# Kamino666/video_features

Hardware: NVIDIA H100
Metric: frames/sec CLIP-ViT-B/32 @224px (higher is better)
Workload: dtype f16

## Files before the change

### video_features_b200/csrc/common.cuh

```cuda
#pragma once
#include <cuda.h>
#include <cuda_runtime.h>
#include <cuda_fp16.h>
#include <stdint.h>

namespace vf {

__device__ __forceinline__ uint32_t smem_u32(const void* p) {
    return static_cast<uint32_t>(__cvta_generic_to_shared(p));
}

__device__ __forceinline__ void mbar_init(uint64_t* bar, uint32_t count) {
    asm volatile("mbarrier.init.shared::cta.b64 [%0], %1;" ::"r"(smem_u32(bar)), "r"(count));
}
__device__ __forceinline__ void fence_mbar_init() {
    asm volatile("fence.mbarrier_init.release.cluster;" ::: "memory");
}
__device__ __forceinline__ void mbar_expect_tx(uint64_t* bar, uint32_t bytes) {
    asm volatile("mbarrier.arrive.expect_tx.shared::cta.b64 _, [%0], %1;" ::"r"(smem_u32(bar)), "r"(bytes)
                 : "memory");
}
__device__ __forceinline__ void mbar_arrive(uint64_t* bar) {
    asm volatile("mbarrier.arrive.shared::cta.b64 _, [%0];" ::"r"(smem_u32(bar)) : "memory");
}
__device__ __forceinline__ void mbar_wait(uint64_t* bar, uint32_t parity) {
    asm volatile(
        "{\n"
        ".reg .pred P1;\n"
        "LAB_WAIT:\n"
        "mbarrier.try_wait.parity.shared::cta.b64 P1, [%0], %1;\n"
        "@P1 bra DONE;\n"
        "bra LAB_WAIT;\n"
        "DONE:\n"
        "}" ::"r"(smem_u32(bar)),
        "r"(parity)
        : "memory");
}

__device__ __forceinline__ void tma_prefetch_desc(const CUtensorMap* tm) {
    asm volatile("prefetch.tensormap [%0];" ::"l"(reinterpret_cast<uint64_t>(tm)) : "memory");
}
__device__ __forceinline__ void tma_load_2d(void* smem_dst, const CUtensorMap* tm, uint64_t* bar, int c0, int c1) {
    asm volatile(
        "cp.async.bulk.tensor.2d.shared::cluster.global.mbarrier::complete_tx::bytes [%0], [%1, {%3, %4}], [%2];" ::"r"(
            smem_u32(smem_dst)),
        "l"(reinterpret_cast<uint64_t>(tm)), "r"(smem_u32(bar)), "r"(c0), "r"(c1)
        : "memory");
}
__device__ __forceinline__ void tma_load_4d(void* smem_dst, const CUtensorMap* tm, uint64_t* bar, int c0, int c1,
                                            int c2, int c3) {
    asm volatile(
        "cp.async.bulk.tensor.4d.shared::cluster.global.mbarrier::complete_tx::bytes [%0], [%1, {%3, %4, %5, %6}], "
        "[%2];" ::"r"(smem_u32(smem_dst)),
        "l"(reinterpret_cast<uint64_t>(tm)), "r"(smem_u32(bar)), "r"(c0), "r"(c1), "r"(c2), "r"(c3)
        : "memory");
}
__device__ __forceinline__ void tma_load_5d(void* smem_dst, const CUtensorMap* tm, uint64_t* bar, int c0, int c1,
                                            int c2, int c3, int c4) {
    asm volatile(
        "cp.async.bulk.tensor.5d.shared::cluster.global.mbarrier::complete_tx::bytes [%0], [%1, {%3, %4, %5, %6, "
        "%7}], [%2];" ::"r"(smem_u32(smem_dst)),
        "l"(reinterpret_cast<uint64_t>(tm)), "r"(smem_u32(bar)), "r"(c0), "r"(c1), "r"(c2), "r"(c3), "r"(c4)
        : "memory");
}

__device__ __forceinline__ void tma_store_2d(const CUtensorMap* tm, const void* smem_src, int c0, int c1) {
    asm volatile("cp.async.bulk.tensor.2d.global.shared::cta.bulk_group [%0, {%2, %3}], [%1];" ::"l"(
                     reinterpret_cast<uint64_t>(tm)),
                 "r"(smem_u32(smem_src)), "r"(c0), "r"(c1)
                 : "memory");
}
__device__ __forceinline__ void tma_reduce_add_2d(const CUtensorMap* tm, const void* smem_src, int c0, int c1) {
    asm volatile("cp.reduce.async.bulk.tensor.2d.global.shared::cta.add.tile.bulk_group [%0, {%2, %3}], [%1];" ::"l"(
                     reinterpret_cast<uint64_t>(tm)),
                 "r"(smem_u32(smem_src)), "r"(c0), "r"(c1)
                 : "memory");
}
__device__ __forceinline__ void red_add_f32x4(float* gptr, float4 v) {
    asm volatile("red.global.add.v4.f32 [%0], {%1, %2, %3, %4};" ::"l"(gptr), "f"(v.x), "f"(v.y), "f"(v.z), "f"(v.w) : "memory");
}
__device__ __forceinline__ void bulk_commit() { asm volatile("cp.async.bulk.commit_group;" ::: "memory"); }
template <int N>
__device__ __forceinline__ void bulk_wait_read() {
    asm volatile("cp.async.bulk.wait_group.read %0;" ::"n"(N) : "memory");
}
template <int N>
__device__ __forceinline__ void bulk_wait() {
    asm volatile("cp.async.bulk.wait_group %0;" ::"n"(N) : "memory");
}
__device__ __forceinline__ void st_shared_b32(uint32_t addr, uint32_t v) {
    asm volatile("st.shared.b32 [%0], %1;" ::"r"(addr), "r"(v) : "memory");
}
__device__ __forceinline__ void st_shared_v2_f32(uint32_t addr, float x, float y) {
    asm volatile("st.shared.v2.f32 [%0], {%1, %2};" ::"r"(addr), "f"(x), "f"(y) : "memory");
}
__device__ __forceinline__ void fence_proxy_async() { asm volatile("fence.proxy.async.shared::cta;" ::: "memory"); }
__device__ __forceinline__ void named_bar_sync(uint32_t id, uint32_t nthreads) {
    asm volatile("bar.sync %0, %1;" ::"r"(id), "r"(nthreads) : "memory");
}
__device__ __forceinline__ void named_bar_arrive(uint32_t id, uint32_t nthreads) {
    asm volatile("bar.arrive %0, %1;" ::"r"(id), "r"(nthreads) : "memory");
}
template <uint32_t N>
__device__ __forceinline__ void setmaxnreg_dec() {
    asm volatile("setmaxnreg.dec.sync.aligned.u32 %0;" ::"n"(N));
}
template <uint32_t N>
__device__ __forceinline__ void setmaxnreg_inc() {
    asm volatile("setmaxnreg.inc.sync.aligned.u32 %0;" ::"n"(N));
}

__device__ __forceinline__ uint64_t wgmma_desc_sw128(const void* smem_tile) {
    uint64_t d = 0;
    d |= static_cast<uint64_t>((smem_u32(smem_tile) & 0x3FFFF) >> 4);
    d |= static_cast<uint64_t>(1) << 16;
    d |= static_cast<uint64_t>(1024 >> 4) << 32;
    d |= static_cast<uint64_t>(1) << 62;
    return d;
}
__device__ __forceinline__ void wgmma_fence() { asm volatile("wgmma.fence.sync.aligned;" ::: "memory"); }
__device__ __forceinline__ void wgmma_commit() { asm volatile("wgmma.commit_group.sync.aligned;" ::: "memory"); }
template <int N>
__device__ __forceinline__ void wgmma_wait() {
    asm volatile("wgmma.wait_group.sync.aligned %0;" ::"n"(N) : "memory");
}
template <int R>
__device__ __forceinline__ void wgmma_fence_regs(float* d) {
#pragma unroll
    for (int i = 0; i < R; ++i) asm volatile("" : "+f"(d[i])::"memory");
}

__device__ __forceinline__ float warp_sum(float v) {
#pragma unroll
    for (int o = 16; o > 0; o >>= 1) v += __shfl_xor_sync(0xffffffffu, v, o);
    return v;
}
__device__ __forceinline__ float warp_max(float v) {
#pragma unroll
    for (int o = 16; o > 0; o >>= 1) v = fmaxf(v, __shfl_xor_sync(0xffffffffu, v, o));
    return v;
}
__device__ __forceinline__ uint32_t pack_half2(float a, float b) {
    __half2 h = __floats2half2_rn(a, b);
    return *reinterpret_cast<uint32_t*>(&h);
}

}
```

### video_features_b200/csrc/gemm.cu

```cuda
#include "gemm_kernel.cuh"

namespace vf {

extern template int launch_bn<1, false, true>(GEMM_LAUNCH_ARGS);
extern template int launch_bn<1, true, true>(GEMM_LAUNCH_ARGS);
extern template int launch_bn<1, false, false>(GEMM_LAUNCH_ARGS);
extern template int launch_bn<1, true, false>(GEMM_LAUNCH_ARGS);
extern template int launch_bn<2, false, false>(GEMM_LAUNCH_ARGS);
extern template int launch_bn<2, true, false>(GEMM_LAUNCH_ARGS);

namespace {

typedef CUresult (*EncodeTiledFn)(CUtensorMap*, CUtensorMapDataType, cuuint32_t, void*, const cuuint64_t*,
                                  const cuuint64_t*, const cuuint32_t*, const cuuint32_t*, CUtensorMapInterleave,
                                  CUtensorMapSwizzle, CUtensorMapL2promotion, CUtensorMapFloatOOBfill);

EncodeTiledFn get_encode_tiled() {
    static EncodeTiledFn fn = nullptr;
    if (fn) return fn;
    void* p = nullptr;
    cudaDriverEntryPointQueryResult q;
    if (cudaGetDriverEntryPoint("cuTensorMapEncodeTiled", &p, cudaEnableDefault, &q) != cudaSuccess ||
        q != cudaDriverEntryPointSuccess)
        return nullptr;
    fn = reinterpret_cast<EncodeTiledFn>(p);
    return fn;
}

}

int device_sm_count() {
    static std::atomic<int> sms[64];
    int dev = 0;
    if (cudaGetDevice(&dev) != cudaSuccess || dev < 0 || dev >= 64) return 132;
    int v = sms[dev].load(std::memory_order_relaxed);
    if (v == 0) {
        if (cudaDeviceGetAttribute(&v, cudaDevAttrMultiProcessorCount, dev) != cudaSuccess || v <= 0) v = 132;
        sms[dev].store(v, std::memory_order_relaxed);
    }
    return v;
}

int make_tmap_2d(CUtensorMap* out, const void* base, int elem_bytes, uint64_t rows, uint64_t cols,
                 uint64_t row_pitch_bytes, uint32_t box_rows, uint32_t box_cols) {
    EncodeTiledFn enc = get_encode_tiled();
    if (!enc) return fail(VF_ERR_CUDA, "cuTensorMapEncodeTiled entry point unavailable (no CUDA driver?)");
    if ((reinterpret_cast<uintptr_t>(base) & 15) || (row_pitch_bytes & 15))
        return fail(VF_ERR_INVALID, "TMA operand must be 16-byte aligned with a 16-byte multiple row pitch");
    if (box_cols * uint32_t(elem_bytes) != 128) return fail(VF_ERR_INVALID, "TMA box rows must be 128 bytes");
    const CUtensorMapDataType dt = elem_bytes == 2 ? CU_TENSOR_MAP_DATA_TYPE_FLOAT16 : CU_TENSOR_MAP_DATA_TYPE_FLOAT32;
    cuuint64_t dims[2] = {cols, rows};
    cuuint64_t strides[1] = {row_pitch_bytes};
    cuuint32_t box[2] = {box_cols, box_rows};
    cuuint32_t estr[2] = {1, 1};
    CUresult r = enc(out, dt, 2, const_cast<void*>(base), dims, strides, box, estr, CU_TENSOR_MAP_INTERLEAVE_NONE,
                     CU_TENSOR_MAP_SWIZZLE_128B, CU_TENSOR_MAP_L2_PROMOTION_L2_256B, CU_TENSOR_MAP_FLOAT_OOB_FILL_NONE);
    if (r != CUDA_SUCCESS) return fail(VF_ERR_CUDA, "cuTensorMapEncodeTiled failed with CUresult %d", int(r));
    return VF_OK;
}

struct GemmProf {
    bool on = false;
    std::vector<cudaEvent_t> ev;
    size_t used = 0;
    double flops = 0.0;
};
static thread_local GemmProf g_prof;

template <bool PP>
static int run_gemm_launch(const CUtensorMap& tmA, const CUtensorMap& tmB, const CUtensorMap& tmD,
                           const CUtensorMap& tmD2, int bn, const GemmEpi& ep, int M, int N, const ConvGeom& cg,
                           cudaStream_t stream) {
    const bool split = ep.split_off > 0 && !ep.out_f32;
    if constexpr (!PP) {
        if (cg.nsplit == 2)
            return split ? launch_bn<2, true, PP>(tmA, tmB, tmD, tmD2, bn, ep, M, N, cg, stream)
                         : launch_bn<2, false, PP>(tmA, tmB, tmD, tmD2, bn, ep, M, N, cg, stream);
    }
    return split ? launch_bn<1, true, PP>(tmA, tmB, tmD, tmD2, bn, ep, M, N, cg, stream)
                 : launch_bn<1, false, PP>(tmA, tmB, tmD, tmD2, bn, ep, M, N, cg, stream);
}

static int run_gemm(const CUtensorMap& tmA, bool pp, const __half* B, int ldb, int64_t Ktot, int M, int N,
                    const ConvGeom& cg, const GemmEpi& ep, cudaStream_t stream) {
    if (!ep.out) return fail(VF_ERR_INVALID, "gemm: null output");
    if (reinterpret_cast<uintptr_t>(ep.out) & 15) return fail(VF_ERR_INVALID, "gemm: output must be 16-byte aligned");
    if (ep.accumulate && !ep.out_f32) return fail(VF_ERR_INVALID, "gemm: accumulate needs fp32 output");
    if (N % 8) return fail(VF_ERR_INVALID, "gemm: N=%d must be a multiple of 8", N);
    if (ep.act < VF_ACT_NONE || ep.act > VF_ACT_GELU) return fail(VF_ERR_INVALID, "gemm: unknown activation %d", ep.act);
    if (ep.out_f32 ? (ep.ldo % 4) : (ep.ldo % 8)) return fail(VF_ERR_INVALID, "gemm: ldo breaks 16-byte rows");
    if (ep.split_off && (ep.out_f32 || ep.split_off < N || ep.split_off % 8))
        return fail(VF_ERR_INVALID, "gemm: split output needs fp16 out and split_off >= N, multiple of 8");
    const int bm = tile_rows(pp);
    const int64_t num_m = (M + bm - 1) / bm, sms = device_sm_count();
    int bn = 256;
    int64_t best = INT64_MAX;
    for (int cand : {256, 192, 128, 64}) {
        const int64_t cost = (num_m * ((N + cand - 1) / cand) + sms - 1) / sms * cand;
        if (cost < best) { best = cost; bn = cand; }
    }
    CUtensorMap tmB, tmD, tmD2;
    VF_TRY(make_tmap_2d(&tmB, B, 2, uint64_t(N), uint64_t(Ktot), uint64_t(ldb) * 2, uint32_t(bn), BK));
    const int eb = ep.out_f32 ? 4 : 2;
    VF_TRY(make_tmap_2d(&tmD, ep.out, eb, uint64_t(M), uint64_t(N), uint64_t(ep.ldo) * eb, EPI_ROWS, 128 / eb));
    if (ep.split_off)
        VF_TRY(make_tmap_2d(&tmD2, static_cast<__half*>(ep.out) + ep.split_off, eb, uint64_t(M), uint64_t(N),
                            uint64_t(ep.ldo) * eb, EPI_ROWS, 128 / eb));
    else
        tmD2 = tmD;
    auto launch = [&] {
        return pp ? run_gemm_launch<true>(tmA, tmB, tmD, tmD2, bn, ep, M, N, cg, stream)
                  : run_gemm_launch<false>(tmA, tmB, tmD, tmD2, bn, ep, M, N, cg, stream);
    };
    if (!g_prof.on) return launch();
    if (g_prof.used + 2 > g_prof.ev.size())
        for (int i = 0; i < 2; ++i) {
            cudaEvent_t e;
            VF_CUDA(cudaEventCreate(&e));
            g_prof.ev.push_back(e);
        }
    VF_CUDA(cudaEventRecord(g_prof.ev[g_prof.used], stream));
    const int st = launch();
    VF_CUDA(cudaEventRecord(g_prof.ev[g_prof.used + 1], stream));
    g_prof.used += 2;
    double kexec = double(Ktot);
    if (cg.nsplit == 2 && cg.lo_mask) {
        const int kpt = (cg.k_per_tap + BK - 1) / BK;
        int skipped = 0;
        for (int kk = 0; kk < kpt && kk < 64; ++kk) skipped += int((cg.lo_mask >> kk) & 1ull);
        kexec -= double(cg.ntaps) * skipped * BK;
    }
    g_prof.flops += 2.0 * double(M) * double(N) * kexec;
    return st;
}

bool gemm_profile_on() { return g_prof.on; }
int gemm_profile(int enable) {
    g_prof.on = enable != 0;
    return VF_OK;
}
int gemm_profile_read(double* ms, int64_t* launches, double* flops) {
    VF_CUDA(cudaDeviceSynchronize());
    double t = 0.0;
    for (size_t i = 0; i + 1 < g_prof.used; i += 2) {
        float x = 0.f;
        VF_CUDA(cudaEventElapsedTime(&x, g_prof.ev[i], g_prof.ev[i + 1]));
        t += x;
    }
    if (ms) *ms = t;
    if (launches) *launches = int64_t(g_prof.used / 2);
    if (flops) *flops = g_prof.flops;
    g_prof.used = 0;
    g_prof.flops = 0.0;
    return VF_OK;
}

int gemm_f16(const __half* A, int lda, const __half* B, int ldb, int M, int N, int K, const GemmEpi& ep,
             cudaStream_t stream) {
    if (M <= 0 || N <= 0 || K <= 0) return fail(VF_ERR_INVALID, "gemm: empty problem %dx%dx%d", M, N, K);
    if (K % 8 || lda % 8 || ldb % 8) return fail(VF_ERR_INVALID, "gemm: K/lda/ldb must be multiples of 8");
    ConvGeom cg;
    memset(&cg, 0, sizeof(cg));
    cg.ntaps = 1;
    cg.k_per_tap = K;
    cg.nsplit = 1;
    CUtensorMap tmA;
    VF_TRY(make_tmap_2d(&tmA, A, 2, uint64_t(M), uint64_t(K), uint64_t(lda) * 2, tile_rows(true), BK));
    return run_gemm(tmA, true, B, ldb, K, M, N, cg, ep, stream);
}

int conv_gemm_f16(const __half* X, int C, int64_t P, const __half* Wt, int N, const ConvGeom& g, const GemmEpi& ep,
                  cudaStream_t stream) {
    if (P <= 0 || P > 0x7fffffff || N <= 0 || C <= 0) return fail(VF_ERR_INVALID, "conv_gemm: bad size");
    if (C % 8) return fail(VF_ERR_INVALID, "conv_gemm: C=%d must be a multiple of 8", C);
    if (g.ntaps < 1 || g.ntaps > 64 || g.k_per_tap < 8 || g.k_per_tap % 8)
        return fail(VF_ERR_INVALID, "conv_gemm: bad tap geometry (%d taps x %d)", g.ntaps, g.k_per_tap);
    if (g.nsplit != 1 && g.nsplit != 2) return fail(VF_ERR_INVALID, "conv_gemm: nsplit must be 1 or 2");
    const int kpt = (g.k_per_tap + BK - 1) / BK;
    if (g.lo_mask && (kpt > 64 || (kpt < 64 && (g.lo_mask >> kpt) != 0)))
        return fail(VF_ERR_INVALID, "conv_gemm: lo_mask 0x%llx names K blocks beyond the %d of a tap", g.lo_mask, kpt);
    if (g.mask && (g.Tp < 1 || g.Hp < 1 || g.Wp < 1 || g.row0 < 0))
        return fail(VF_ERR_INVALID, "conv_gemm: bad mask volume %dx%dx%d, row0 %d", g.Tp, g.Hp, g.Wp, g.row0);
    CUtensorMap tmA;
    VF_TRY(make_tmap_2d(&tmA, X, 2, uint64_t(P), uint64_t(g.k_per_tap), uint64_t(C) * 2, tile_rows(false), BK));
    const int64_t Ktot = int64_t(g.ntaps) * g.k_per_tap * g.nsplit;
    if (Ktot % 8) return fail(VF_ERR_INVALID, "conv_gemm: K must be a multiple of 8");
    return run_gemm(tmA, false, Wt, int(Ktot), Ktot, int(P), N, g, ep, stream);
}

}
```

### video_features_b200/csrc/gemm_inst_pp.cu

```cuda
#include "gemm_kernel.cuh"

namespace vf {
template int launch_bn<1, false, true>(GEMM_LAUNCH_ARGS);
template int launch_bn<1, true, true>(GEMM_LAUNCH_ARGS);
}
```

### video_features_b200/csrc/gemm_kernel.cuh

```cuda
#pragma once
#include <stdarg.h>
#include <stdlib.h>
#include <string.h>

#include <atomic>
#include <vector>

#include "common.cuh"
#include "internal.h"
#include "wgmma.cuh"

namespace vf {

namespace {

constexpr int BK = 64;
constexpr int THREADS = 384;
constexpr uint32_t PRODUCER_REGS = 40, CONSUMER_REGS = 232;
constexpr int EPI_ROWS = 64;
constexpr uint32_t STG_BYTES = EPI_ROWS * 128;
constexpr uint32_t STAGING_BYTES = 2 * 2 * STG_BYTES;
constexpr uint32_t SMEM_LIMIT = 227 * 1024;
constexpr uint32_t MAX_STAGES = 8;
constexpr uint32_t RING_BUDGET = SMEM_LIMIT - STAGING_BYTES - 2 * MAX_STAGES * 8 - 1024;

template <int BN, int NSPLIT, bool PP>
struct GemmCfg {
    static constexpr int BM = PP ? 64 : 128;
    static constexpr uint32_t A_BYTES = BM * BK * 2;
    static constexpr uint32_t B_TILE = BN * BK * 2;
    static constexpr uint32_t B_BYTES = NSPLIT * B_TILE;
    static constexpr uint32_t STAGE_BYTES = A_BYTES + B_BYTES;
    static constexpr int STAGES = RING_BUDGET / STAGE_BYTES > MAX_STAGES ? MAX_STAGES : int(RING_BUDGET / STAGE_BYTES);
    static constexpr uint32_t BAR_BYTES = 2 * STAGES * 8;
    static constexpr uint32_t SMEM_BYTES = STAGES * STAGE_BYTES + STAGING_BYTES + BAR_BYTES + 1024;
    static_assert(STAGES >= 2, "at least two pipeline stages");
    static_assert(SMEM_BYTES <= SMEM_LIMIT, "shared memory budget");
    static_assert(A_BYTES % 1024 == 0 && B_TILE % 1024 == 0, "swizzle-128B tiles must stay 1024-byte aligned");
};

constexpr int tile_rows(bool pp) { return pp ? GemmCfg<64, 1, true>::BM : GemmCfg<64, 1, false>::BM; }

template <int ACT>
__device__ __forceinline__ float apply_act(float v) {
    if (ACT == VF_ACT_QUICKGELU) {
        return __fdividef(v, 1.0f + __expf(-1.702f * v));
    } else if (ACT == VF_ACT_RELU) {
        return fmaxf(v, 0.0f);
    } else if (ACT == VF_ACT_SIGMOID) {
        return __fdividef(1.0f, 1.0f + __expf(-v));
    } else if (ACT == VF_ACT_TANH) {
        return 1.0f - __fdividef(2.0f, 1.0f + __expf(2.0f * v));
    } else if (ACT == VF_ACT_LEAKY) {
        return v > 0.0f ? v : __fmul_rn(v, 0.1f);
    } else if (ACT == VF_ACT_GELU) {
        return 0.5f * v * (1.0f + erff(v * 0.70710678118654752f));
    }
    return v;
}

template <int BN, int NSPLIT, bool SPLIT, bool PP, int ACT>
__global__ void __launch_bounds__(THREADS, 1)
gemm_f16_kernel(const __grid_constant__ CUtensorMap tmA, const __grid_constant__ CUtensorMap tmB,
                const __grid_constant__ CUtensorMap tmD, const __grid_constant__ CUtensorMap tmD2, const GemmEpi ep,
                const int M, const int N, const __grid_constant__ ConvGeom cg) {
    using Cfg = GemmCfg<BN, NSPLIT, PP>;
    static_assert(PP ? NSPLIT == 1 : true, "split weights run in the conv mode only");
    constexpr int STAGES = Cfg::STAGES;
    constexpr int BM = Cfg::BM;
    extern __shared__ uint8_t smem_raw[];
    uint8_t* smem = reinterpret_cast<uint8_t*>((reinterpret_cast<uintptr_t>(smem_raw) + 1023) & ~uintptr_t(1023));
    uint8_t* sA = smem;
    uint8_t* sB = smem + STAGES * Cfg::A_BYTES;
    uint8_t* sD = smem + STAGES * Cfg::STAGE_BYTES;
    uint64_t* full = reinterpret_cast<uint64_t*>(sD + STAGING_BYTES);
    uint64_t* empty = full + STAGES;

    const int warp = threadIdx.x >> 5;
    const int lane = threadIdx.x & 31;
    const int num_m = (M + BM - 1) / BM;
    const int num_n = (N + BN - 1) / BN;
    const int num_tiles = num_m * num_n;
    auto tile_m0 = [&](int tile) { return (PP ? tile / num_n : tile % num_m) * BM; };
    auto tile_n0 = [&](int tile) { return (PP ? tile % num_n : tile / num_m) * BN; };
    const int cta_tiles = (num_tiles - 1 - int(blockIdx.x)) / int(gridDim.x) + 1;
    const int kpt = (cg.k_per_tap + BK - 1) / BK;
    const int num_k = cg.ntaps * kpt;

    if (threadIdx.x == 0) {
        tma_prefetch_desc(&tmA);
        tma_prefetch_desc(&tmB);
        tma_prefetch_desc(&tmD);
        if (SPLIT) tma_prefetch_desc(&tmD2);
        for (int i = 0; i < STAGES; ++i) {
            mbar_init(&full[i], 1);
            mbar_init(&empty[i], PP ? 4 : 8);
        }
        fence_mbar_init();
    }
    __syncthreads();

    if (warp < 4) {
        setmaxnreg_dec<PRODUCER_REGS>();
        if (warp == 0 && lane == 0) {
            int stage = 0;
            uint32_t phase = 0;
            for (int i = 0; i < cta_tiles; ++i) {
                const int tile = blockIdx.x + i * gridDim.x;
                const int m0 = tile_m0(tile), n0 = tile_n0(tile);
                for (int tap = 0; tap < cg.ntaps; ++tap) {
                    const int arow = m0 + cg.tap_off[tap];
                    const int bcol = tap * cg.k_per_tap;
                    for (int kk = 0; kk < kpt; ++kk) {
                        mbar_wait(&empty[stage], phase ^ 1);
                        const bool lo_blk = NSPLIT == 2 && ((cg.lo_mask >> kk) & 1ull);
                        mbar_expect_tx(&full[stage], Cfg::A_BYTES + (lo_blk ? Cfg::B_TILE : Cfg::B_BYTES));
                        tma_load_2d(sA + stage * Cfg::A_BYTES, &tmA, &full[stage], kk * BK, arow);
                        tma_load_2d(sB + stage * Cfg::B_BYTES, &tmB, &full[stage], bcol + kk * BK, n0);
                        if (NSPLIT == 2 && !lo_blk)
                            tma_load_2d(sB + stage * Cfg::B_BYTES + Cfg::B_TILE, &tmB, &full[stage],
                                        cg.ntaps * cg.k_per_tap + bcol + kk * BK, n0);
                        if (++stage == STAGES) { stage = 0; phase ^= 1; }
                    }
                }
            }
        }
        return;
    }

    setmaxnreg_inc<CONSUMER_REGS>();
    const int wg = (warp >> 2) - 1;
    const int wq = warp & 3;
    constexpr int R = BN / 2;
    float acc[R];
    const bool issuer = (threadIdx.x & 127) == 0;
    uint32_t buf = 0;
    auto wg_sync = [&] {
        if (wg == 0) named_bar_sync(1, 128);
        else named_bar_sync(2, 128);
    };
    auto store_subtile = [&](int col, int row) {
        fence_proxy_async();
        if (issuer) bulk_wait_read<0>();
        wg_sync();
        if (issuer) {
            const uint8_t* src = sD + (wg * 2 + buf) * STG_BYTES;
            if (ep.accumulate) tma_reduce_add_2d(&tmD, src, col, row);
            else tma_store_2d(&tmD, src, col, row);
            bulk_commit();
        }
        buf ^= 1;
    };
    auto wait_turn = [&] {
        if (wg == 0) named_bar_sync(3, 256);
        else named_bar_sync(4, 256);
    };
    auto pass_turn = [&] {
        if (wg == 0) named_bar_arrive(4, 256);
        else named_bar_arrive(3, 256);
    };
    for (int i = PP ? wg : 0; i < cta_tiles; i += PP ? 2 : 1) {
        const int tile = blockIdx.x + i * gridDim.x;
        const int m0 = tile_m0(tile) + (PP ? 0 : wg * 64), n0 = tile_n0(tile);
        const uint64_t first = uint64_t(i) * uint64_t(num_k);
        int stage = int(first % STAGES);
        uint32_t phase = uint32_t(first / STAGES) & 1u;
        if (PP && i > 0) wait_turn();
        int prev = -1;
        for (int kb = 0, kk = 0; kb < num_k; ++kb) {
            mbar_wait(&full[stage], phase);
            const uint64_t adesc = wgmma_desc_sw128(sA + stage * Cfg::A_BYTES + (PP ? 0 : wg * (64 * 128)));
            const uint64_t bdesc = wgmma_desc_sw128(sB + stage * Cfg::B_BYTES);
            const bool lo_blk = NSPLIT == 2 && ((cg.lo_mask >> kk) & 1ull);
            wgmma_fence_regs<R>(acc);
            wgmma_fence();
#pragma unroll
            for (int k = 0; k < BK / 16; ++k) {
                Wgmma<BN>::mma(acc, adesc + 2 * k, bdesc + 2 * k, (kb | k) != 0 ? 1u : 0u);
                if (NSPLIT == 2 && !lo_blk) Wgmma<BN>::mma(acc, adesc + 2 * k, bdesc + (Cfg::B_TILE >> 4) + 2 * k, 1u);
            }
            wgmma_commit();
            wgmma_wait<1>();
            wgmma_fence_regs<R>(acc);
            if (prev >= 0) {
                __syncwarp();
                if (lane == 0) mbar_arrive(&empty[prev]);
            }
            prev = stage;
            if (++stage == STAGES) { stage = 0; phase ^= 1; }
            if (++kk == kpt) kk = 0;
        }
        if (PP && i + 1 < cta_tiles) pass_turn();
        float2 sc[8], bi[8];
        auto load_sb = [&](int s) {
#pragma unroll
            for (int c = 0; c < 8; ++c) {
                const int n = min(n0 + 64 * s + 8 * c + 2 * (lane & 3), N - 2);
                sc[c] = ep.scale ? __ldg(reinterpret_cast<const float2*>(ep.scale + n)) : make_float2(1.f, 1.f);
                bi[c] = ep.bias ? __ldg(reinterpret_cast<const float2*>(ep.bias + n)) : make_float2(-0.f, -0.f);
            }
        };
        load_sb(0);
        wgmma_wait<0>();
        wgmma_fence_regs<R>(acc);
        __syncwarp();
        if (lane == 0) mbar_arrive(&empty[prev]);

        bool keep[2] = {true, true};
        if (cg.mask) {
#pragma unroll
            for (int h = 0; h < 2; ++h) {
                const int mm = m0 + wq * 16 + (lane >> 2) + 8 * h - cg.row0;
                const int w = mm % cg.Wp, r1 = mm / cg.Wp;
                const int hh = r1 % cg.Hp, r2 = r1 / cg.Hp;
                const int tt = r2 % cg.Tp;
                keep[h] = (mm >= 0) && (w >= cg.w0) && (w < cg.w1) && (hh >= cg.h0) && (hh < cg.h1) && (tt >= cg.t0) && (tt < cg.t1);
            }
        }
        const int row = m0;
        const uint32_t stg = smem_u32(sD) + wg * 2 * STG_BYTES + (wq * 16 + (lane >> 2)) * 128;
        const int swz = lane >> 2;
#pragma unroll
        for (int s = 0; s < BN / 64; ++s) {
            if (n0 + 64 * s >= N) break;
#pragma unroll
            for (int c = 0; c < 8; ++c)
#pragma unroll
                for (int h = 0; h < 2; ++h) {
                    const int j = 8 * s + c;
                    float v0 = __fadd_rn(__fmul_rn(acc[4 * j + 2 * h], sc[c].x), bi[c].x);
                    float v1 = __fadd_rn(__fmul_rn(acc[4 * j + 2 * h + 1], sc[c].y), bi[c].y);
                    v0 = apply_act<ACT>(v0);
                    v1 = apply_act<ACT>(v1);
                    acc[4 * j + 2 * h] = keep[h] ? v0 : 0.f;
                    acc[4 * j + 2 * h + 1] = keep[h] ? v1 : 0.f;
                }
            if (s + 1 < BN / 64) load_sb(s + 1);
            if (SPLIT) {
                if (issuer) bulk_wait_read<0>();
                wg_sync();
#pragma unroll
                for (int c = 0; c < 8; ++c)
#pragma unroll
                    for (int h = 0; h < 2; ++h) {
                        const int j = 8 * s + c;
                        const float v0 = acc[4 * j + 2 * h], v1 = acc[4 * j + 2 * h + 1];
                        const __half2 hi = __floats2half2_rn(v0, v1);
                        const uint32_t off = h * 8 * 128 + ((c ^ swz) << 4) + 4 * (lane & 3);
                        st_shared_b32(stg + off, *reinterpret_cast<const uint32_t*>(&hi));
                        st_shared_b32(stg + STG_BYTES + off, pack_half2(v0 - __low2float(hi), v1 - __high2float(hi)));
                    }
                fence_proxy_async();
                wg_sync();
                if (issuer) {
                    tma_store_2d(&tmD, sD + wg * 2 * STG_BYTES, n0 + 64 * s, row);
                    tma_store_2d(&tmD2, sD + (wg * 2 + 1) * STG_BYTES, n0 + 64 * s, row);
                    bulk_commit();
                }
            } else if (ep.out_f32) {
#pragma unroll
                for (int q = 0; q < 2; ++q) {
                    if (q == 1 && n0 + 64 * s + 32 >= N) break;
                    const uint32_t d = stg + buf * STG_BYTES;
#pragma unroll
                    for (int c = 0; c < 4; ++c) {
                        const int j = 8 * s + 4 * q + c;
                        const int chunk = 2 * c + ((lane & 3) >> 1);
#pragma unroll
                        for (int h = 0; h < 2; ++h)
                            st_shared_v2_f32(d + h * 8 * 128 + ((chunk ^ swz) << 4) + 8 * (lane & 1), acc[4 * j + 2 * h],
                                             acc[4 * j + 2 * h + 1]);
                    }
                    store_subtile(n0 + 64 * s + 32 * q, row);
                }
            } else {
                const uint32_t d = stg + buf * STG_BYTES;
#pragma unroll
                for (int c = 0; c < 8; ++c)
#pragma unroll
                    for (int h = 0; h < 2; ++h) {
                        const int j = 8 * s + c;
                        st_shared_b32(d + h * 8 * 128 + ((c ^ swz) << 4) + 4 * (lane & 3),
                                      pack_half2(acc[4 * j + 2 * h], acc[4 * j + 2 * h + 1]));
                    }
                store_subtile(n0 + 64 * s, row);
            }
        }
    }
    if (issuer) bulk_wait<0>();
}

template <int BN, int NSPLIT, bool SPLIT, bool PP, int ACT>
int launch_gemm(const CUtensorMap& tmA, const CUtensorMap& tmB, const CUtensorMap& tmD, const CUtensorMap& tmD2,
                const GemmEpi& ep, int M, int N, const ConvGeom& cg, cudaStream_t stream) {
    using Cfg = GemmCfg<BN, NSPLIT, PP>;
    static std::atomic<bool> attr_set[64];
    int dev = 0;
    VF_CUDA(cudaGetDevice(&dev));
    if (dev < 0 || dev >= 64 || !attr_set[dev].load(std::memory_order_acquire)) {
        VF_CUDA(cudaFuncSetAttribute(gemm_f16_kernel<BN, NSPLIT, SPLIT, PP, ACT>,
                                     cudaFuncAttributeMaxDynamicSharedMemorySize, Cfg::SMEM_BYTES));
        if (dev >= 0 && dev < 64) attr_set[dev].store(true, std::memory_order_release);
    }
    const int tiles = ((M + Cfg::BM - 1) / Cfg::BM) * ((N + BN - 1) / BN);
    const int sms = device_sm_count();
    const int grid = tiles < sms ? tiles : sms;
    gemm_f16_kernel<BN, NSPLIT, SPLIT, PP, ACT><<<grid, THREADS, Cfg::SMEM_BYTES, stream>>>(tmA, tmB, tmD, tmD2, ep, M,
                                                                                            N, cg);
    VF_CUDA(cudaGetLastError());
    return VF_OK;
}

template <int BN, int NSPLIT, bool SPLIT, bool PP>
int launch_act(const CUtensorMap& tmA, const CUtensorMap& tmB, const CUtensorMap& tmD, const CUtensorMap& tmD2,
               const GemmEpi& ep, int M, int N, const ConvGeom& cg, cudaStream_t stream) {
    switch (ep.act) {
        case VF_ACT_QUICKGELU:
            return launch_gemm<BN, NSPLIT, SPLIT, PP, VF_ACT_QUICKGELU>(tmA, tmB, tmD, tmD2, ep, M, N, cg, stream);
        case VF_ACT_RELU:
            return launch_gemm<BN, NSPLIT, SPLIT, PP, VF_ACT_RELU>(tmA, tmB, tmD, tmD2, ep, M, N, cg, stream);
        case VF_ACT_SIGMOID:
            return launch_gemm<BN, NSPLIT, SPLIT, PP, VF_ACT_SIGMOID>(tmA, tmB, tmD, tmD2, ep, M, N, cg, stream);
        case VF_ACT_TANH:
            return launch_gemm<BN, NSPLIT, SPLIT, PP, VF_ACT_TANH>(tmA, tmB, tmD, tmD2, ep, M, N, cg, stream);
        case VF_ACT_LEAKY:
            if constexpr (NSPLIT == 2 && !PP)
                return launch_gemm<BN, NSPLIT, SPLIT, PP, VF_ACT_LEAKY>(tmA, tmB, tmD, tmD2, ep, M, N, cg, stream);
            else
                return fail(VF_ERR_INVALID, "gemm: LeakyReLU is built for split-weight convolutions (nsplit = 2) only");
        case VF_ACT_GELU:
            if constexpr (!SPLIT && ((NSPLIT == 1 && PP) || (NSPLIT == 2 && !PP)))
                return launch_gemm<BN, NSPLIT, SPLIT, PP, VF_ACT_GELU>(tmA, tmB, tmD, tmD2, ep, M, N, cg, stream);
            else
                return fail(VF_ERR_INVALID, "gemm: GELU is built for gemm_f16 and split-weight convolutions, without split output, only");
        default:
            return launch_gemm<BN, NSPLIT, SPLIT, PP, VF_ACT_NONE>(tmA, tmB, tmD, tmD2, ep, M, N, cg, stream);
    }
}

}

#define GEMM_LAUNCH_ARGS                                                                                           \
    const CUtensorMap &tmA, const CUtensorMap &tmB, const CUtensorMap &tmD, const CUtensorMap &tmD2, int bn,       \
        const GemmEpi &ep, int M, int N, const ConvGeom &cg, cudaStream_t stream
template <int NSPLIT, bool SPLIT, bool PP>
int launch_bn(GEMM_LAUNCH_ARGS) {
    if (bn == 256) return launch_act<256, NSPLIT, SPLIT, PP>(tmA, tmB, tmD, tmD2, ep, M, N, cg, stream);
    if (bn == 192) return launch_act<192, NSPLIT, SPLIT, PP>(tmA, tmB, tmD, tmD2, ep, M, N, cg, stream);
    if (bn == 128) return launch_act<128, NSPLIT, SPLIT, PP>(tmA, tmB, tmD, tmD2, ep, M, N, cg, stream);
    return launch_act<64, NSPLIT, SPLIT, PP>(tmA, tmB, tmD, tmD2, ep, M, N, cg, stream);
}

}
```

Baseline: 46040.

## Multicast B tiles across 2-CTA clusters in ping-pong GEMM

Launches the ping-pong GEMM as 2-CTA clusters that work on adjacent M tiles sharing the same N tile. Each CTA TMA-loads half of the B tile and multicasts it to both CTAs, which halves B global/L2 traffic per pair. Empty barriers now take arrivals from both CTAs through remote mbarrier arrives, and cluster syncs are added at start and exit. In exchange, the tile scheduler works at pair granularity and tile-width selection uses a cluster occupancy query, which can cause imbalance when the M tile count is odd and adds coupling between the two CTAs.

Result: no change. 46620, median of 6 (+1.3%).

```diff
diff --git a/video_features_b200/csrc/common.cuh b/video_features_b200/csrc/common.cuh
--- a/video_features_b200/csrc/common.cuh
+++ b/video_features_b200/csrc/common.cuh
@@ -36,6 +36,26 @@
         "r"(parity)
         : "memory");
 }
+__device__ __forceinline__ void mbar_arrive_cluster_relaxed(uint64_t* bar, uint32_t cta) {
+    asm volatile(
+        "{\n"
+        ".reg .b32 ra;\n"
+        "mapa.shared::cluster.u32 ra, %0, %1;\n"
+        "mbarrier.arrive.relaxed.cluster.shared::cluster.b64 _, [ra];\n"
+        "}" ::"r"(smem_u32(bar)),
+        "r"(cta)
+        : "memory");
+}
+
+__device__ __forceinline__ uint32_t cluster_ctarank() {
+    uint32_t r;
+    asm volatile("mov.u32 %0, %%cluster_ctarank;" : "=r"(r));
+    return r;
+}
+__device__ __forceinline__ void cluster_sync() {
+    asm volatile("barrier.cluster.arrive.release;\n"
+                 "barrier.cluster.wait.acquire;" ::: "memory");
+}
 
 __device__ __forceinline__ void tma_prefetch_desc(const CUtensorMap* tm) {
     asm volatile("prefetch.tensormap [%0];" ::"l"(reinterpret_cast<uint64_t>(tm)) : "memory");
@@ -45,6 +65,14 @@
         "cp.async.bulk.tensor.2d.shared::cluster.global.mbarrier::complete_tx::bytes [%0], [%1, {%3, %4}], [%2];" ::"r"(
             smem_u32(smem_dst)),
         "l"(reinterpret_cast<uint64_t>(tm)), "r"(smem_u32(bar)), "r"(c0), "r"(c1)
+        : "memory");
+}
+__device__ __forceinline__ void tma_load_2d_multicast(void* smem_dst, const CUtensorMap* tm, uint64_t* bar, int c0, int c1,
+                                                      uint16_t cta_mask) {
+    asm volatile(
+        "cp.async.bulk.tensor.2d.shared::cluster.global.mbarrier::complete_tx::bytes.multicast::cluster [%0], [%1, {%3, "
+        "%4}], [%2], %5;" ::"r"(smem_u32(smem_dst)),
+        "l"(reinterpret_cast<uint64_t>(tm)), "r"(smem_u32(bar)), "r"(c0), "r"(c1), "h"(cta_mask)
         : "memory");
 }
 __device__ __forceinline__ void tma_load_4d(void* smem_dst, const CUtensorMap* tm, uint64_t* bar, int c0, int c1,
diff --git a/video_features_b200/csrc/gemm.cu b/video_features_b200/csrc/gemm.cu
--- a/video_features_b200/csrc/gemm.cu
+++ b/video_features_b200/csrc/gemm.cu
@@ -92,15 +92,22 @@
     if (ep.split_off && (ep.out_f32 || ep.split_off < N || ep.split_off % 8))
         return fail(VF_ERR_INVALID, "gemm: split output needs fp16 out and split_off >= N, multiple of 8");
     const int bm = tile_rows(pp);
-    const int64_t num_m = (M + bm - 1) / bm, sms = device_sm_count();
+    const int64_t num_m = (M + bm - 1) / bm;
     int bn = 256;
     int64_t best = INT64_MAX;
     for (int cand : {256, 192, 128, 64}) {
-        const int64_t cost = (num_m * ((N + cand - 1) / cand) + sms - 1) / sms * cand;
+        int64_t row_units = num_m, slots = device_sm_count();
+        if (pp) {
+            int c = 0;
+            VF_TRY(gemm_pp_cluster_slots(cand, &c));
+            row_units = (num_m + 1) / 2;
+            slots = c;
+        }
+        const int64_t cost = (row_units * ((N + cand - 1) / cand) + slots - 1) / slots * cand;
         if (cost < best) { best = cost; bn = cand; }
     }
     CUtensorMap tmB, tmD, tmD2;
-    VF_TRY(make_tmap_2d(&tmB, B, 2, uint64_t(N), uint64_t(Ktot), uint64_t(ldb) * 2, uint32_t(bn), BK));
+    VF_TRY(make_tmap_2d(&tmB, B, 2, uint64_t(N), uint64_t(Ktot), uint64_t(ldb) * 2, uint32_t(pp ? bn / 2 : bn), BK));
     const int eb = ep.out_f32 ? 4 : 2;
     VF_TRY(make_tmap_2d(&tmD, ep.out, eb, uint64_t(M), uint64_t(N), uint64_t(ep.ldo) * eb, EPI_ROWS, 128 / eb));
     if (ep.split_off)
diff --git a/video_features_b200/csrc/gemm_inst_pp.cu b/video_features_b200/csrc/gemm_inst_pp.cu
--- a/video_features_b200/csrc/gemm_inst_pp.cu
+++ b/video_features_b200/csrc/gemm_inst_pp.cu
@@ -3,4 +3,50 @@
 namespace vf {
 template int launch_bn<1, false, true>(GEMM_LAUNCH_ARGS);
 template int launch_bn<1, true, true>(GEMM_LAUNCH_ARGS);
+
+namespace {
+
+template <int BN>
+int query_pp_cluster_slots(int* slots) {
+    using Cfg = GemmCfg<BN, 1, true>;
+    auto kernel = gemm_f16_kernel<BN, 1, false, true, VF_ACT_NONE>;
+    VF_CUDA(cudaFuncSetAttribute(kernel, cudaFuncAttributeMaxDynamicSharedMemorySize, Cfg::SMEM_BYTES));
+    cudaLaunchAttribute attr[1];
+    attr[0].id = cudaLaunchAttributeClusterDimension;
+    attr[0].val.clusterDim.x = 2;
+    attr[0].val.clusterDim.y = 1;
+    attr[0].val.clusterDim.z = 1;
+    cudaLaunchConfig_t lc = {};
+    lc.gridDim = dim3(2);
+    lc.blockDim = dim3(THREADS);
+    lc.dynamicSmemBytes = Cfg::SMEM_BYTES;
+    lc.attrs = attr;
+    lc.numAttrs = 1;
+    VF_CUDA(cudaOccupancyMaxActiveClusters(slots, kernel, &lc));
+    if (*slots < 1) return fail(VF_ERR_CUDA, "gemm: no 2-CTA cluster of the BN = %d ping-pong kernel fits on the device", BN);
+    return VF_OK;
 }
+
+}
+
+int gemm_pp_cluster_slots(int bn, int* slots) {
+    static std::atomic<int> cache[64][4];
+    int dev = 0;
+    VF_CUDA(cudaGetDevice(&dev));
+    const int w = bn / 64 - 1;
+    if (bn % 64 || w < 0 || w > 3) return fail(VF_ERR_INVALID, "gemm: no ping-pong tile width %d", bn);
+    int v = dev >= 0 && dev < 64 ? cache[dev][w].load(std::memory_order_relaxed) : 0;
+    if (v == 0) {
+        switch (bn) {
+            case 256: VF_TRY(query_pp_cluster_slots<256>(&v)); break;
+            case 192: VF_TRY(query_pp_cluster_slots<192>(&v)); break;
+            case 128: VF_TRY(query_pp_cluster_slots<128>(&v)); break;
+            default: VF_TRY(query_pp_cluster_slots<64>(&v)); break;
+        }
+        if (dev >= 0 && dev < 64) cache[dev][w].store(v, std::memory_order_relaxed);
+    }
+    *slots = v;
+    return VF_OK;
+}
+
+}
diff --git a/video_features_b200/csrc/gemm_kernel.cuh b/video_features_b200/csrc/gemm_kernel.cuh
--- a/video_features_b200/csrc/gemm_kernel.cuh
+++ b/video_features_b200/csrc/gemm_kernel.cuh
@@ -11,6 +11,8 @@
 #include "wgmma.cuh"
 
 namespace vf {
+
+int gemm_pp_cluster_slots(int bn, int* slots);
 
 namespace {
 
@@ -80,10 +82,13 @@
     const int lane = threadIdx.x & 31;
     const int num_m = (M + BM - 1) / BM;
     const int num_n = (N + BN - 1) / BN;
-    const int num_tiles = num_m * num_n;
-    auto tile_m0 = [&](int tile) { return (PP ? tile / num_n : tile % num_m) * BM; };
+    const int rank = PP ? int(cluster_ctarank()) : 0;
+    const int unit = PP ? int(blockIdx.x) >> 1 : int(blockIdx.x);
+    const int units = PP ? int(gridDim.x) >> 1 : int(gridDim.x);
+    const int num_tiles = PP ? (num_m + 1) / 2 * num_n : num_m * num_n;
+    auto tile_m0 = [&](int tile) { return (PP ? 2 * (tile / num_n) + rank : tile % num_m) * BM; };
     auto tile_n0 = [&](int tile) { return (PP ? tile % num_n : tile / num_m) * BN; };
-    const int cta_tiles = (num_tiles - 1 - int(blockIdx.x)) / int(gridDim.x) + 1;
+    const int cta_tiles = (num_tiles - 1 - unit) / units + 1;
     const int kpt = (cg.k_per_tap + BK - 1) / BK;
     const int num_k = cg.ntaps * kpt;
 
@@ -94,11 +99,12 @@
         if (SPLIT) tma_prefetch_desc(&tmD2);
         for (int i = 0; i < STAGES; ++i) {
             mbar_init(&full[i], 1);
-            mbar_init(&empty[i], PP ? 4 : 8);
+            mbar_init(&empty[i], 8);
         }
         fence_mbar_init();
     }
-    __syncthreads();
+    if (PP) cluster_sync();
+    else __syncthreads();
 
     if (warp < 4) {
         setmaxnreg_dec<PRODUCER_REGS>();
@@ -106,7 +112,7 @@
             int stage = 0;
             uint32_t phase = 0;
             for (int i = 0; i < cta_tiles; ++i) {
-                const int tile = blockIdx.x + i * gridDim.x;
+                const int tile = unit + i * units;
                 const int m0 = tile_m0(tile), n0 = tile_n0(tile);
                 for (int tap = 0; tap < cg.ntaps; ++tap) {
                     const int arow = m0 + cg.tap_off[tap];
@@ -116,7 +122,11 @@
                         const bool lo_blk = NSPLIT == 2 && ((cg.lo_mask >> kk) & 1ull);
                         mbar_expect_tx(&full[stage], Cfg::A_BYTES + (lo_blk ? Cfg::B_TILE : Cfg::B_BYTES));
                         tma_load_2d(sA + stage * Cfg::A_BYTES, &tmA, &full[stage], kk * BK, arow);
-                        tma_load_2d(sB + stage * Cfg::B_BYTES, &tmB, &full[stage], bcol + kk * BK, n0);
+                        if (PP)
+                            tma_load_2d_multicast(sB + stage * Cfg::B_BYTES + rank * (Cfg::B_TILE / 2), &tmB, &full[stage],
+                                                  bcol + kk * BK, n0 + rank * (BN / 2), 0x3);
+                        else
+                            tma_load_2d(sB + stage * Cfg::B_BYTES, &tmB, &full[stage], bcol + kk * BK, n0);
                         if (NSPLIT == 2 && !lo_blk)
                             tma_load_2d(sB + stage * Cfg::B_BYTES + Cfg::B_TILE, &tmB, &full[stage],
                                         cg.ntaps * cg.k_per_tap + bcol + kk * BK, n0);
@@ -125,6 +135,7 @@
                 }
             }
         }
+        if (PP) cluster_sync();
         return;
     }
 
@@ -159,8 +170,15 @@
         if (wg == 0) named_bar_arrive(4, 256);
         else named_bar_arrive(3, 256);
     };
+    auto release = [&](int s) {
+        __syncwarp();
+        if (lane == 0) {
+            mbar_arrive(&empty[s]);
+            if (PP) mbar_arrive_cluster_relaxed(&empty[s], uint32_t(rank ^ 1));
+        }
+    };
     for (int i = PP ? wg : 0; i < cta_tiles; i += PP ? 2 : 1) {
-        const int tile = blockIdx.x + i * gridDim.x;
+        const int tile = unit + i * units;
         const int m0 = tile_m0(tile) + (PP ? 0 : wg * 64), n0 = tile_n0(tile);
         const uint64_t first = uint64_t(i) * uint64_t(num_k);
         int stage = int(first % STAGES);
@@ -182,10 +200,7 @@
             wgmma_commit();
             wgmma_wait<1>();
             wgmma_fence_regs<R>(acc);
-            if (prev >= 0) {
-                __syncwarp();
-                if (lane == 0) mbar_arrive(&empty[prev]);
-            }
+            if (prev >= 0) release(prev);
             prev = stage;
             if (++stage == STAGES) { stage = 0; phase ^= 1; }
             if (++kk == kpt) kk = 0;
@@ -203,8 +218,7 @@
         load_sb(0);
         wgmma_wait<0>();
         wgmma_fence_regs<R>(acc);
-        __syncwarp();
-        if (lane == 0) mbar_arrive(&empty[prev]);
+        release(prev);
 
         bool keep[2] = {true, true};
         if (cg.mask) {
@@ -288,6 +302,7 @@
         }
     }
     if (issuer) bulk_wait<0>();
+    if (PP) cluster_sync();
 }
 
 template <int BN, int NSPLIT, bool SPLIT, bool PP, int ACT>
@@ -302,7 +317,27 @@
                                      cudaFuncAttributeMaxDynamicSharedMemorySize, Cfg::SMEM_BYTES));
         if (dev >= 0 && dev < 64) attr_set[dev].store(true, std::memory_order_release);
     }
-    const int tiles = ((M + Cfg::BM - 1) / Cfg::BM) * ((N + BN - 1) / BN);
+    const int num_m = (M + Cfg::BM - 1) / Cfg::BM, num_n = (N + BN - 1) / BN;
+    if constexpr (PP) {
+        int slots = 0;
+        VF_TRY(gemm_pp_cluster_slots(BN, &slots));
+        const int pairs = (num_m + 1) / 2 * num_n;
+        cudaLaunchAttribute attr[1];
+        attr[0].id = cudaLaunchAttributeClusterDimension;
+        attr[0].val.clusterDim.x = 2;
+        attr[0].val.clusterDim.y = 1;
+        attr[0].val.clusterDim.z = 1;
+        cudaLaunchConfig_t lc = {};
+        lc.gridDim = dim3(2 * (pairs < slots ? pairs : slots));
+        lc.blockDim = dim3(THREADS);
+        lc.dynamicSmemBytes = Cfg::SMEM_BYTES;
+        lc.stream = stream;
+        lc.attrs = attr;
+        lc.numAttrs = 1;
+        VF_CUDA(cudaLaunchKernelEx(&lc, gemm_f16_kernel<BN, NSPLIT, SPLIT, PP, ACT>, tmA, tmB, tmD, tmD2, ep, M, N, cg));
+        return VF_OK;
+    }
+    const int tiles = num_m * num_n;
     const int sms = device_sm_count();
     const int grid = tiles < sms ? tiles : sms;
     gemm_f16_kernel<BN, NSPLIT, SPLIT, PP, ACT><<<grid, THREADS, Cfg::SMEM_BYTES, stream>>>(tmA, tmB, tmD, tmD2, ep, M,
```
